# haoheliu/ssr_eval

Measured on AMD Instinct MI355X. Metric: utterance-pairs/sec (LSD+SSIM, 48kHz, n_fft=2048), higher is better.
Workload: dtype f64

## Files before the change

### ssr_eval_amd/csrc/ssr_stft_wave.h

```cpp
#pragma once
#include "ssr_stft.h"


constexpr int SSR_W_N = 2048, SSR_W_L = 64, SSR_W_P = 32;
constexpr int SSR_W_TWP = 7 * 32 + 12 * 64;
SSR_DEV int ssr_wpad(int i) { return i + (i >> 5); }
constexpr int SSR_W_PN = SSR_W_N + (SSR_W_N >> 5) + 1;

template <typename T> SSR_DEV cx<T> ssr_w32(int m) {
  constexpr double c[22] = {1.0, 0.98078528040323044913, 0.92387953251128675613, 0.83146961230254523708, 0.70710678118654752440,
                            0.55557023301960222474, 0.38268343236508977173, 0.19509032201612826785, 0.0,
                            -0.19509032201612826785, -0.38268343236508977173, -0.55557023301960222474, -0.70710678118654752440,
                            -0.83146961230254523708, -0.92387953251128675613, -0.98078528040323044913, -1.0,
                            -0.98078528040323044913, -0.92387953251128675613, -0.83146961230254523708, -0.70710678118654752440,
                            -0.55557023301960222474};
  constexpr double s[22] = {0.0, -0.19509032201612826785, -0.38268343236508977173, -0.55557023301960222474, -0.70710678118654752440,
                            -0.83146961230254523708, -0.92387953251128675613, -0.98078528040323044913, -1.0,
                            -0.98078528040323044913, -0.92387953251128675613, -0.83146961230254523708, -0.70710678118654752440,
                            -0.55557023301960222474, -0.38268343236508977173, -0.19509032201612826785, 0.0,
                            0.19509032201612826785, 0.38268343236508977173, 0.55557023301960222474, 0.70710678118654752440,
                            0.83146961230254523708};
  return {(T)c[m], (T)s[m]};
}

template <typename T, int NZ = 32> SSR_DEV void ssr_dft32(cx<T>* v) {
  const T h = (T)0.70710678118654752440;
  static_assert(NZ == 32 || (NZ > 8 && NZ <= 16), "full, or two non-zero row groups");
  SSR_UNROLL for (int n2 = 0; n2 < 8; ++n2) {
    cx<T> t[4] = {v[n2], v[8 + n2], v[16 + n2], v[24 + n2]};
    if (NZ == 32) {
      ssr_bfly4(t);
    } else if (8 + n2 < NZ) {
      const cx<T> r = cmul_negi(t[1]);
      t[2] = csub(t[0], t[1]); t[3] = csub(t[0], r);
      t[1] = cadd(t[0], r);    t[0] = cadd(t[0], v[8 + n2]);
    } else {
      t[1] = t[0]; t[2] = t[0]; t[3] = t[0];
    }
    SSR_UNROLL for (int k1 = 0; k1 < 4; ++k1) {
      const int m = n2 * k1;
      cx<T> x = t[k1];
      if (m == 0) {
      } else if (m == 8) {
        x = cmul_negi(x);
      } else if (m == 16) {
        x = {-x.x, -x.y};
      } else if (m == 4) {
        x = {h * (x.x + x.y), h * (x.y - x.x)};
      } else if (m == 12) {
        x = {h * (x.y - x.x), -h * (x.x + x.y)};
      } else if (m == 20) {
        x = {-h * (x.x + x.y), h * (x.x - x.y)};
      } else {
        x = cmul(x, ssr_w32<T>(m));
      }
      v[8 * k1 + n2] = x;
    }
  }
  SSR_UNROLL for (int k1 = 0; k1 < 4; ++k1) ssr_bfly8(v + 8 * k1);
}
SSR_DEV constexpr int ssr_dft32_freq(int rho) { return (rho >> 3) + 4 * (rho & 7); }

struct SsrTrue { static constexpr bool value = true; };
struct SsrFalse { static constexpr bool value = false; };

template <typename T, bool SUMS> struct SsrWaveRegs {
  cx<T> v[SSR_W_P];
  T tx[SSR_W_P];
  float pa[SSR_W_P], pb[SSR_W_P];
  T wl[SSR_W_P / 2];
  cx<T> tw1[3];
  cx<T> tw2[12];
  double lsd_total;
};

template <typename T, bool SPLIT> struct SsrWaveLds {
  static constexpr size_t bytes() { return sizeof(double) * 4 + sizeof(int) * 8 + sizeof(T) * (SPLIT ? 1 : 2) * SSR_W_PN; }
  double* sc1; int* nz; T* re; T* im;
  SSR_MEMBER explicit SsrWaveLds(char* base) {
    sc1 = reinterpret_cast<double*>(base);
    nz = reinterpret_cast<int*>(sc1 + 4);
    re = reinterpret_cast<T*>(nz + 8);
    im = SPLIT ? re : re + SSR_W_PN;
  }
  SSR_MEMBER bool nonzero(int which, int par) const {
    int f = nz[which * 2 + par];
#ifndef SSR_HOST_EMU
    f = __builtin_amdgcn_readfirstlane(f);
#endif
    return f != 0;
  }
};

template <typename T> struct SsrWaveBuf { T* re; T* im; };

template <typename T, bool SPLIT> constexpr size_t ssr_stft_wave_sums_offset() { return (SsrWaveLds<T, SPLIT>::bytes() + 7) & ~(size_t)7; }
template <typename T, bool SPLIT, bool SUMS> constexpr size_t ssr_stft_wave_lds_bytes() {
  return SUMS ? ssr_stft_wave_sums_offset<T, SPLIT>() + 6 * 64 * sizeof(double) : SsrWaveLds<T, SPLIT>::bytes();
}

struct SsrWaveBase { int st0, ld8, st1; };
SSR_DEV SsrWaveBase ssr_wave_bases(int tid) {
  return {33 * tid, tid + (tid >> 5), 264 * (tid >> 5) + (tid & 31)};
}
SSR_DEV constexpr int ssr_w_off_st0(int i) { return ssr_dft32_freq(i); }
SSR_DEV constexpr int ssr_w_off_ld8(int i) { return 66 * (i >> 3) + 264 * (i & 7); }
SSR_DEV constexpr int ssr_w_off_st1(int i) { return 528 * (i >> 3) + 33 * (i & 7); }

#define SSR_W_EXCHANGE_G(blk, regs, L, WB, WO, RBASES, RIDX, EXTRA)                                       \
  if constexpr (!SPLIT) {                                                                                 \
    SSR_WPHASE(blk, regs, { const int w_ = ssr_wave_bases(tid & 63).WB;                                        \
      SSR_UNROLL for (int i = 0; i < SSR_W_P; ++i) { (L).re[w_ + WO(i)] = R.v[i].x; (L).im[w_ + WO(i)] = R.v[i].y; } }); \
    SSR_WPHASE(blk, regs, { SSR_SCHED_BARRIER(); EXTRA; const auto r_ = RBASES(tid & 63);                    \
      SSR_UNROLL for (int i = 0; i < SSR_W_P; ++i) R.v[i] = {(L).re[RIDX(r_, i)], (L).im[RIDX(r_, i)]}; });   \
  } else {                                                                                                \
    SSR_WPHASE(blk, regs, { const int w_ = ssr_wave_bases(tid & 63).WB;                                        \
      SSR_UNROLL for (int i = 0; i < SSR_W_P; ++i) (L).re[w_ + WO(i)] = R.v[i].x; });                     \
    SSR_WPHASE(blk, regs, { SSR_SCHED_BARRIER(); EXTRA; const auto r_ = RBASES(tid & 63);                    \
      SSR_UNROLL for (int i = 0; i < SSR_W_P; ++i) R.tx[i] = (L).re[RIDX(r_, i)]; });                     \
    SSR_WPHASE(blk, regs, { const int w_ = ssr_wave_bases(tid & 63).WB;                                        \
      SSR_UNROLL for (int i = 0; i < SSR_W_P; ++i) (L).re[w_ + WO(i)] = R.v[i].y; });                     \
    SSR_WPHASE(blk, regs, { const auto r_ = RBASES(tid & 63);                                                \
      SSR_UNROLL for (int i = 0; i < SSR_W_P; ++i) R.v[i] = {R.tx[i], (L).re[RIDX(r_, i)]}; });           \
  }
#define SSR_W_RIDX_LD8(b_, i) ((b_).ld8 + ssr_w_off_ld8(i))
#define SSR_W_EXCHANGE(blk, regs, L, WB, WO, RB, RO, EXTRA) SSR_W_EXCHANGE_G(blk, regs, L, WB, WO, ssr_wave_bases, SSR_W_RIDX_##RB##_##RO, EXTRA)
#define SSR_W_RIDX_ld8_ssr_w_off_ld8(b_, i) SSR_W_RIDX_LD8(b_, i)

struct SsrWavePBase { int ld8, p2, p3; };
SSR_DEV int ssr_wave_pj3(int tid) { return tid == 0 ? 128 : 256 - tid; }
SSR_DEV SsrWavePBase ssr_wave_pbases(int tid) {
  return {tid + (tid >> 5), ssr_wpad(192 - tid), ssr_wpad(ssr_wave_pj3(tid))};
}
SSR_DEV int ssr_w_rd_paired(const SsrWavePBase& B, int i) {
  const int b = i >> 3, q = i & 7;
  return (b == 0 ? B.ld8 : b == 1 ? B.ld8 + 66 : b == 2 ? B.p2 : B.p3) + 264 * q;
}
#define SSR_W_RIDX_PAIRED(b_, i) ssr_w_rd_paired(b_, i)
#define SSR_W_LOAD_TW2_PAIRED { const int t_ = tid & 63; const unsigned l_ = SSR_UIDX(t_);                       \
    const unsigned o2_ = SSR_UIDX(t_ == 0 ? 192 : 64 - t_); const unsigned o3_ = SSR_UIDX(t_ == 0 ? -192 : 64 - t_); \
    SSR_UNROLL for (int i = 0; i < 6; ++i) R.tw2[i] = VT.at(l_ + (SSR_W_N + 224 + 64 * i));                       \
    SSR_UNROLL for (int i = 6; i < 9; ++i) R.tw2[i] = VT.at(o2_ + (SSR_W_N + 224 + 64 * i));                      \
    SSR_UNROLL for (int i = 9; i < 12; ++i) R.tw2[i] = VT.at(o3_ + (SSR_W_N + 224 + 64 * i)); }

#define SSR_W_LOAD_TW1 { const unsigned l_ = SSR_UIDX(tid & 31); \
                         SSR_UNROLL for (int m = 0; m < 3; ++m) R.tw1[m] = VT.at(l_ + (SSR_W_N + 32 * ((1 << m) - 1))); }
#define SSR_W_LOAD_TW2 { const unsigned l_ = SSR_UIDX(tid & 63); \
                         SSR_UNROLL for (int i = 0; i < 12; ++i) R.tw2[i] = VT.at(l_ + (SSR_W_N + 224 + 64 * i)); }
#define SSR_W_FFT_TAIL(blk, BLK0, regs, L, EXTRA2)                                                                        \
  SSR_W_FFT_TAIL_X(blk, BLK0, regs, L, SSR_W_EXCHANGE(blk, regs, L, st1, ssr_w_off_st1, ld8, ssr_w_off_ld8, SSR_W_LOAD_TW2 EXTRA2))
#define SSR_W_FFT_TAIL_PAIRED(blk, BLK0, regs, L)                                                                         \
  SSR_W_FFT_TAIL_X(blk, BLK0, regs, L, SSR_W_EXCHANGE_G(blk, regs, L, st1, ssr_w_off_st1, ssr_wave_pbases, SSR_W_RIDX_PAIRED, SSR_W_LOAD_TW2_PAIRED))
#define SSR_W_FFT_TAIL_X(blk, BLK0, regs, L, EXCH2)                                                                   \
  blk = BLK0; ssr_launder(blk);                                                                                       \
  SSR_W_EXCHANGE(blk, regs, L, st0, ssr_w_off_st0, ld8, ssr_w_off_ld8, SSR_W_LOAD_TW1);                               \
  \
  SSR_WPHASE(blk, regs, {                                                                                             \
    const cx<T> s1_ = ssr_tw_w8(R.tw1[0]);                                                                            \
    SSR_UNROLL for (int b = 0; b < 4; ++b) ssr_bfly8_tw(R.v + 8 * b, R.tw1[0], R.tw1[1], R.tw1[2], s1_);              \
  });                                                                                                                 \
  blk = BLK0; ssr_launder(blk);                                                                                       \
  EXCH2;                                                                                                              \
                     \
  SSR_WPHASE(blk, regs, {                                                                                             \
    SSR_UNROLL for (int b = 0; b < 4; ++b)                                                                            \
      ssr_bfly8_tw(R.v + 8 * b, R.tw2[3 * b], R.tw2[3 * b + 1], R.tw2[3 * b + 2], ssr_tw_w8(R.tw2[3 * b]));           \
  });

template <typename T, int WHICH = 3, typename REGS>
SSR_DEV void ssr_wave_prefetch(const SsrStftParams<T>& p, REGS& R, int tid, const SsrView<float>& va, const SsrView<float>& vb,
                               int u, int n, int n_frames) {
  const int t_c = (u < n_frames) ? u : n_frames - 1;
  const int base = t_c * p.hop - SSR_W_N / 2;
  if (base >= 0 && base + SSR_W_N <= n) {
    SSR_UNROLL for (int r = 0; r < SSR_W_P; ++r) {
      if (WHICH & 1) R.pa[r] = va.at(SSR_UIDX(tid + 64 * r), base);
      if (WHICH & 2) R.pb[r] = vb.at(SSR_UIDX(tid + 64 * r), base);
    }
  } else {
    SSR_UNROLL for (int r = 0; r < SSR_W_P; ++r) {
      const unsigned m = SSR_UIDX(ssr_reflect(base + tid + 64 * r, n));
      if (WHICH & 1) R.pa[r] = va.at(m);
      if (WHICH & 2) R.pb[r] = vb.at(m);
    }
  }
}

template <typename REGS> SSR_DEV void ssr_wave_flags(REGS& R, int tid, int* nz, int par) {
  SSR_UNROLL for (int r = 0; r < SSR_W_P; ++r) { ssr_touch(R.pa[r]); ssr_touch(R.pb[r]); }
  unsigned ora = 0u, orb = 0u;
  SSR_UNROLL for (int r = 1; r < SSR_W_P; ++r) { ora |= ssr_mag_bits(R.pa[r]); orb |= ssr_mag_bits(R.pb[r]); }
  ora |= (tid == 0) ? 0u : ssr_mag_bits(R.pa[0]);
  orb |= (tid == 0) ? 0u : ssr_mag_bits(R.pb[0]);
  SSR_WAVE_ANY_STORE(tid, ora != 0u, nz + par);
  SSR_WAVE_ANY_STORE(tid, orb != 0u, nz + 2 + par);
}

template <typename T, bool SUMS, bool SPLIT, int MAG = -1, typename BLK>
SSR_BODY void ssr_stft_wave_body(const SsrStftParams<T>& p, BLK& blk, int chunk, int item, char* lds_base) {
  constexpr int N = SSR_W_N, F = N / 2 + 1;
  using Regs = SsrWaveRegs<T, SUMS>;
  SsrWaveLds<T, SPLIT> L(lds_base);
  const int n = p.len[item], hop = p.hop;
  const int n_frames = ssr_num_frames_dev(n, N, hop);
  const int S = p.interleave > 1 ? p.interleave : 1;
  const int span0 = (chunk / S) * S * p.units_per_chunk;
  const int u0 = span0 + chunk % S;
  const int u1 = (span0 + S * p.units_per_chunk < n_frames) ? span0 + S * p.units_per_chunk : n_frames;
  const float* sa = p.a + p.a_off[item];
  const float* sb = p.b + p.b_off[item];
  const int64_t row0 = p.frame_off[item];
  double* part = p.part ? p.part + ((int64_t)item * p.n_chunks + chunk) * SSR_NPART : nullptr;
  const int mask = SUMS ? p.metric_mask : (p.metric_mask & SSR_M_LSD);
  const bool want_lsd = mask & SSR_M_LSD;
  const SsrView<float> va(sa, n), vb(sb, n);
  const SsrView<T> vw(p.window, N);
  const SsrView<cx<T>> vt(p.tw, N + SSR_W_TWP);

  double* lsum = reinterpret_cast<double*>(lds_base + ssr_stft_wave_sums_offset<T, SPLIT>());
  SSR_REGS(Regs, regs, blk);
  SSR_WPHASE(blk, regs, {
    R.lsd_total = 0.0;
    if constexpr (SUMS) for (int q = 0; q < 6; ++q) lsum[64 * q + tid] = 0.0;
    if (tid == 0) L.sc1[0] = 0.0;
    if (u0 < u1) {
      ssr_wave_prefetch<T>(p, R, tid, va, vb, u0, n, n_frames);
      SSR_UNROLL for (int r = 0; r < SSR_W_P / 2; ++r) R.wl[r] = vw.at(SSR_UIDX(tid + 64 * r));
    }
    SSR_VMEM_DRAIN();
  });

  BLK blk0 = blk;
  for (int u = u0, it = 0; u < u1; u += S, ++it) {
    blk = blk0; ssr_launder(blk);
    SSR_WPHASE(blk, regs, {
      ssr_wave_flags(R, tid, L.nz, it & 1);
      SSR_UNROLL for (int r = 0; r < SSR_W_P; ++r) {
        const T w = (r < SSR_W_P / 2) ? R.wl[r] : (T)0.5 - R.wl[r - SSR_W_P / 2];
        R.v[r] = {(T)R.pa[r] * w, (T)R.pb[r] * w};
      }
      ssr_dft32(R.v);
      if (want_lsd && it > 0 && tid == 0) R.lsd_total += sqrt(L.sc1[0] / (double)F);
    });
#define VT vt
    SSR_W_FFT_TAIL_PAIRED(blk, blk0, regs, L);
#undef VT

    blk = blk0; ssr_launder(blk);
    const int64_t OP = p.out_pitch ? p.out_pitch : F;
    float* ra0 = p.out_a ? p.out_a + (row0 + u) * OP : nullptr;
    float* rb0 = p.out_b ? p.out_b + (row0 + u) * OP : nullptr;
    SSR_WPHASE(blk, regs, {
      SSR_SCHED_BARRIER();
      double acc[7] = {0.0, 0.0, 0.0, 0.0, 0.0, 0.0, 0.0};
      const int par = it & 1;
      const bool a_nz = L.nonzero(0, par), b_nz = L.nonzero(1, par);
      const bool both = a_nz && b_nz;
      const bool store = MAG < 0 ? p.out_kind == SSR_OUT_MAG : MAG != 0;
      const SsrRwView<float> wa(ra0, store ? F : 0), wb(rb0, (store && rb0 != nullptr) ? F : 0);
      const int lane4 = 4 * tid, lane4_2 = 4 * (192 - tid), lane4_3 = 4 * ssr_wave_pj3(tid);
      auto bin_off = [&](int b, int q) -> int {
        return (b == 0 ? lane4 : b == 1 ? lane4 + 256 : b == 2 ? lane4_2 : lane4_3) + 1024 * q;
      };
      cx<T> rot4 = {(T)0, (T)0};
      if (tid == 0) {
        rot4 = R.v[28];
        const cx<T> t29 = R.v[29], t30 = R.v[30], t31 = R.v[31];
        R.v[31] = R.v[0]; R.v[30] = R.v[7]; R.v[29] = R.v[6]; R.v[28] = R.v[5];
        R.v[7] = t31; R.v[6] = t30; R.v[5] = t29;
      }
      constexpr int G = 2;
      constexpr int PF1 = SUMS ? 1 : 0;
      auto bins = [&](auto fast_tag) {
        constexpr bool FAST = decltype(fast_tag)::value;
        SSR_UNROLL for (int b = 0; b < 4; ++b) SSR_UNROLL for (int q0 = 0; q0 < 4; q0 += G) {
          cx<T> zn[G];
          SSR_UNROLL for (int q = 0; q < G; ++q) zn[q] = R.v[8 * (3 - b) + 7 - (q0 + q)];
          SSR_UNROLL for (int q = 0; q < G; q += 2) {
            const cx<T> zk0 = R.v[8 * b + q0 + q], zk1 = R.v[8 * b + q0 + q + 1];
            f2 e, t;
            if constexpr (FAST) {
              ssr_pair_bins2_fast<T, SUMS>(acc, zk0, zn[q], zk1, zn[q + 1], e, t);
            } else {
              float e0, t0, e1, t1;
              ssr_pair_bin<T, 0, true>(mask, acc, zk0, zn[q], a_nz, b_nz, e0, t0);
              ssr_pair_bin<T, 0, true>(mask, acc, zk1, zn[q + 1], a_nz, b_nz, e1, t1);
              e = f2_make(e0, e1); t = f2_make(t0, t1);
            }
            if (store) {
              wa.st_raw(bin_off(b, q0 + q), e.x);
              wa.st_raw(bin_off(b, q0 + q + 1), e.y);
              wb.st_raw(bin_off(b, q0 + q), t.x);
              wb.st_raw(bin_off(b, q0 + q + 1), t.y);
            }
          }
          if (b == 0 && q0 + G == 4) {
            if (tid == 0) {
              const cx<T> zq = R.v[4];
              float e, t;
              ssr_pair_bin<T, 0, true>(mask, acc, zq, zq, a_nz, b_nz, e, t);
              if (store) { wa.st_raw(4 * (N / 2), e); wb.st_raw(4 * (N / 2), t); }
              R.v[4] = rot4;
            }
          }
          if (b == PF1 && q0 + G == 4) {
            SSR_SCHED_BARRIER();
            ssr_wave_prefetch<T, 1>(p, R, tid, va, vb, u + S, n, n_frames);
            SSR_SCHED_BARRIER();
          }
          if (b == PF1 + 1 && q0 + G == 4) {
            SSR_SCHED_BARRIER();
            ssr_wave_prefetch<T, 2>(p, R, tid, va, vb, u + S, n, n_frames);
            SSR_SCHED_BARRIER();
          }
          if (b == PF1 + 2 && q0 + G == 4) {
            SSR_SCHED_BARRIER();
            SSR_UNROLL for (int r = 0; r < SSR_W_P / 2; ++r) R.wl[r] = vw.at(SSR_UIDX(tid + 64 * r));
            SSR_SCHED_BARRIER();
          }
        }
      };
      constexpr int FULL = SUMS ? (SSR_M_LSD | SSR_M_LOG_SISPEC | SSR_M_SISPEC) : SSR_M_LSD;
      if (both && (mask & 7) == FULL) bins(SsrTrue{});
      else bins(SsrFalse{});
      if (want_lsd) SSR_WAVE_SUM_STORE(tid, 64, acc[0], L.sc1);
      if constexpr (SUMS)
        for (int q = 0; q < 6; ++q) SSR_LDS_ACCUM(lsum + 64 * q + tid, acc[1 + q]);
    });
  }

  if (part == nullptr) return;
  if constexpr (SUMS) {
    for (int q = 0; q < 6; ++q) {
      SSR_WPHASE(blk, regs, SSR_WAVE_SUM_STORE(tid, 64, lsum[64 * q + tid], L.sc1 + 1));
      SSR_WPHASE(blk, regs, if (tid == 0) part[1 + q] = L.sc1[1]);
    }
  } else {
    SSR_WPHASE(blk, regs, if (tid == 0) for (int q = 0; q < 6; ++q) part[1 + q] = 0.0);
  }
  SSR_WPHASE(blk, regs, if (tid == 0) {
    double lsd = R.lsd_total;
    if (want_lsd && u1 > u0) lsd += sqrt(L.sc1[0] / (double)F);
    part[0] = lsd;
    part[7] = 0.0;
  });
}
```

### ssr_eval_amd/csrc/ssr_tables.h

```cpp
#pragma once
#include <cmath>
#include <cstdint>
#include <vector>

#include "ssr_block.h"

static const long double SSR_PI_L = 3.14159265358979323846264338327950288L;

inline bool ssr_is_pow2(int n) { return n > 0 && (n & (n - 1)) == 0; }
inline int ssr_ilog2(int n) { int l = 0; while ((1 << l) < n) ++l; return l; }

struct SsrEngine { bool ok; bool bluestein; int logn; int radix; int q; int m; };
inline SsrEngine ssr_pick_engine(int n_fft) {
  SsrEngine e{false, false, 0, 1, 0, 0};
  if (n_fft < 2) return e;
  e.q = n_fft;
  if (ssr_is_pow2(n_fft) && n_fft >= 256 && n_fft <= 4096) { e.ok = true; e.logn = ssr_ilog2(n_fft); return e; }
  int m = 256;
  while (m < 2 * n_fft - 1) m <<= 1;
  if (n_fft % 3 == 0 && m >= 8192) {
    const int q = n_fft / 3;
    int mq = 256;
    while (mq < 2 * q - 1) mq <<= 1;
    if (mq <= 2048) { e.ok = true; e.bluestein = true; e.logn = ssr_ilog2(mq); e.radix = 3; e.q = q; return e; }
  }
  if (m > 8192) return e;
  e.ok = true; e.bluestein = true; e.logn = ssr_ilog2(m);
  return e;
}

inline SsrEngine ssr_pick_wave_engine(int n_fft) {
  const SsrEngine e = ssr_pick_engine(n_fft);
  SsrEngine none{false, false, 0, 1, 0, 0};
  if (!e.ok || !e.bluestein) return none;
  SsrEngine w = none;
  if (e.radix == 3) w = (e.logn == 11 && e.q <= 768) ? e : none;
  else if (e.logn == 11) w = e;
  else if (e.logn == 12 && n_fft % 2 == 0 && n_fft / 2 <= 1024) w = SsrEngine{true, true, 11, 2, n_fft / 2, 0};
  if (w.ok && w.q <= 768) w.m = 1536;
  return w;
}

constexpr int SSR_WAVE_N = 2048, SSR_WAVE_TWP = 7 * 32 + 12 * 64;
constexpr int SSR_WAVE24_N = 1536, SSR_WAVE24_TWP = 2 * 9 * 64;

template <typename T> struct SsrTables {
  SsrEngine eng;
  int n_fft;
  std::vector<T> window;
  std::vector<T> window_h;
  std::vector<cx<T>> tw, wchirp, bfilt, chirp;
};

inline void ssr_host_fft_ld(std::vector<long double>& re, std::vector<long double>& im) {
  const int n = (int)re.size();
  for (int i = 1, j = 0; i < n; ++i) {
    int bit = n >> 1;
    for (; j & bit; bit >>= 1) j ^= bit;
    j ^= bit;
    if (i < j) { std::swap(re[i], re[j]); std::swap(im[i], im[j]); }
  }
  for (int len = 2; len <= n; len <<= 1) {
    for (int i = 0; i < n; i += len) {
      for (int k = 0; k < len / 2; ++k) {
        const long double ang = -2.0L * SSR_PI_L * k / len;
        const long double wr = cosl(ang), wi = sinl(ang);
        const int a = i + k, b = i + k + len / 2;
        const long double xr = re[b] * wr - im[b] * wi, xi = re[b] * wi + im[b] * wr;
        re[b] = re[a] - xr; im[b] = im[a] - xi;
        re[a] += xr; im[a] += xi;
      }
    }
  }
}

inline void ssr_host_dft_ld(std::vector<long double>& re, std::vector<long double>& im) {
  const int n = (int)re.size();
  std::vector<long double> c(n), s(n), orr(n), oi(n);
  for (int i = 0; i < n; ++i) { const long double a = -2.0L * SSR_PI_L * i / n; c[i] = cosl(a); s[i] = sinl(a); }
  for (int k = 0; k < n; ++k) {
    long double ar = 0.0L, ai = 0.0L;
    for (int m = 0; m < n; ++m) {
      const int j = (int)(((int64_t)k * m) % n);
      ar += re[m] * c[j] - im[m] * s[j];
      ai += re[m] * s[j] + im[m] * c[j];
    }
    orr[k] = ar; oi[k] = ai;
  }
  re = orr; im = oi;
}

template <typename T> bool ssr_build_tables_for(int n_fft, SsrEngine eng, SsrTables<T>& t);
template <typename T> bool ssr_build_tables(int n_fft, SsrTables<T>& t) { return ssr_build_tables_for<T>(n_fft, ssr_pick_engine(n_fft), t); }

template <typename T> bool ssr_build_tables_for(int n_fft, SsrEngine eng, SsrTables<T>& t) {
  t.eng = eng;
  t.n_fft = n_fft;
  if (!t.eng.ok) return false;
  const int N = t.eng.m ? t.eng.m : (1 << t.eng.logn);
  t.window.resize(n_fft);
  std::vector<long double> w(n_fft);
  for (int m = 0; m < n_fft; ++m) {
    w[m] = 0.5L - 0.5L * cosl(2.0L * SSR_PI_L * m / n_fft);
    t.window[m] = (T)w[m];
  }
  t.window_h.resize(n_fft);
  for (int m = 0; m < n_fft; ++m) t.window_h[m] = (T)0.5 * t.window[m];
  t.tw.resize(N);
  for (int i = 0; i < N; ++i) {
    const long double ang = -2.0L * SSR_PI_L * i / N;
    t.tw[i] = {(T)cosl(ang), (T)sinl(ang)};
  }
  if (N == SSR_WAVE24_N) {
    t.tw.resize(N + SSR_WAVE24_TWP);
    for (int b = 0; b < 3; ++b)
      for (int k = 0; k < 3; ++k)
        for (int l = 0; l < 64; ++l) {
          const int j = l + 64 * b, q = j % 24;
          t.tw[N + 64 * (3 * b + k) + l] = t.tw[(8 * q << k) % N];
          t.tw[N + 576 + 64 * (3 * b + k) + l] = t.tw[(j << k) % N];
        }
  }
  if (N == SSR_WAVE_N) {
    t.tw.resize(N + SSR_WAVE_TWP);
    for (int q = 1; q < 8; ++q)
      for (int l = 0; l < 32; ++l) t.tw[N + 32 * (q - 1) + l] = t.tw[8 * l * q];
    for (int b = 0; b < 4; ++b)
      for (int k = 0; k < 3; ++k)
        for (int l = 0; l < 64; ++l) t.tw[N + 224 + 64 * (3 * b + k) + l] = t.tw[(l + 64 * b) << k];
  }
  if (t.eng.bluestein) {
    const int q = t.eng.q, R = t.eng.radix;
    std::vector<long double> cr(q), ci(q);
    for (int k = 0; k < q; ++k) {
      const int64_t kk = ((int64_t)k * k) % (2 * (int64_t)q);
      const long double ang = -SSR_PI_L * (long double)kk / q;
      cr[k] = cosl(ang); ci[k] = sinl(ang);
    }
    t.chirp.resize((size_t)R * q); t.wchirp.resize((size_t)R * q);
    for (int r = 0; r < R; ++r)
      for (int k = 0; k < q; ++k) {
        const int64_t rk = ((int64_t)r * k) % n_fft;
        const long double a2 = -2.0L * SSR_PI_L * (long double)rk / n_fft;
        const long double tr = cosl(a2), ti = sinl(a2);
        t.chirp[(size_t)r * q + k] = {(T)(0.5L * (cr[k] * tr - ci[k] * ti)), (T)(0.5L * (cr[k] * ti + ci[k] * tr))};
        const long double wv = w[(size_t)R * k + r];
        t.wchirp[(size_t)r * q + k] = {(T)(wv * cr[k]), (T)(wv * ci[k])};
      }
    std::vector<long double> br(N, 0.0L), bi(N, 0.0L);
    for (int m = 0; m < q; ++m) {
      br[m] = cr[m]; bi[m] = -ci[m];
      if (m) { br[N - m] = cr[m]; bi[N - m] = -ci[m]; }
    }
    if (ssr_is_pow2(N)) ssr_host_fft_ld(br, bi); else ssr_host_dft_ld(br, bi);
    t.bfilt.resize(N);
    for (int i = 0; i < N; ++i) t.bfilt[i] = {(T)(br[i] / N), (T)(bi[i] / N)};
  }
  return true;
}
```

### ssr_eval_amd/csrc/tu_stft.inc

```
#include "ssr_host.h"
#include "ssr_stft_r3.h"
#include "ssr_stft_wave.h"
#include "ssr_stft_rn_wave.h"
#include "ssr_stft_r3_rot.h"

typedef SSR_TU_T TT;
static_assert(SSR_W_N == SSR_WAVE_N && SSR_W_TWP == SSR_WAVE_TWP, "ssr_tables.h appends what ssr_stft_wave.h reads");
static_assert(SSR_W24_N == SSR_WAVE24_N && SSR_W24_TWP == SSR_WAVE24_TWP, "ssr_tables.h appends what ssr_fft24.h reads");

constexpr int ssr_stft_min_waves(int logn, bool blu, bool sums) { return (logn == 11 && !blu && !sums) ? 4 : 1; }

#if SSR_TU_PART <= 2
template <typename T, int LOGN, bool BLU, int MODE, bool SUMS, int E64>
__global__ __launch_bounds__((1 << LOGN) / ssr_stft_ppt(LOGN, BLU), E64 ? 1 : ssr_stft_min_waves(LOGN, BLU, SUMS))
void k_stft(SsrStftParams<T> p) {
  extern __shared__ __attribute__((aligned(16))) char smem[];
  SsrBlk blk{(int)threadIdx.x};
  const int item = blockIdx.x / p.n_chunks, chunk = blockIdx.x % p.n_chunks;
  ssr_stft_body<T, LOGN, BLU, MODE, SUMS, ssr_stft_ppt(LOGN, BLU), E64>(p, blk, chunk, item, smem);
}

template <typename T, int LOGN, bool BLU, int MODE, bool SUMS, int E64 = 0>
static int launch_stft_mode(SsrStftParams<T>& p, int grid, hipStream_t s) {
  constexpr int PPT = ssr_stft_ppt(LOGN, BLU);
  const size_t lds = SsrStftLds<T, LOGN, PPT>::bytes();
  static thread_local SsrLdsSlot slot;
  if (int rc = ssr_allow_lds((const void*)k_stft<T, LOGN, BLU, MODE, SUMS, E64>, lds, &slot)) return rc;
  hipLaunchKernelGGL((k_stft<T, LOGN, BLU, MODE, SUMS, E64>), dim3(grid), dim3((1 << LOGN) / PPT), lds, s, p);
  HIP_TRY(hipGetLastError());
  return SSR_OK;
}

template <typename T, int LOGN, bool BLU> static int launch_stft_inst(SsrStftParams<T>& p, int grid, hipStream_t s) {
  const bool sums = p.metric_mask & (SSR_M_SISPEC | SSR_M_LOG_SISPEC);
  (void)sums;
#if SSR_TU_PART == 2
  return launch_stft_mode<T, LOGN, BLU, SSR_MODE_SINGLE, false>(p, grid, s);
#elif SSR_TU_PART == 1
  if (p.a64 && p.b64)
    return sums ? launch_stft_mode<T, LOGN, BLU, SSR_MODE_PAIR, true, SSR_IN_BOTH64>(p, grid, s)
                : launch_stft_mode<T, LOGN, BLU, SSR_MODE_PAIR, false, SSR_IN_BOTH64>(p, grid, s);
  return sums ? launch_stft_mode<T, LOGN, BLU, SSR_MODE_PAIR, true, SSR_IN_EST64>(p, grid, s)
              : launch_stft_mode<T, LOGN, BLU, SSR_MODE_PAIR, false, SSR_IN_EST64>(p, grid, s);
#else
  return sums ? launch_stft_mode<T, LOGN, BLU, SSR_MODE_PAIR, true>(p, grid, s)
              : launch_stft_mode<T, LOGN, BLU, SSR_MODE_PAIR, false>(p, grid, s);
#endif
}

#if SSR_TU_PART == 0
template <typename T, bool SUMS, bool SPLIT, bool MAG>
__global__ __launch_bounds__(64, SPLIT ? 2 : 1) void k_stft_wave(SsrStftParams<T> p, int n_groups) {
  extern __shared__ __attribute__((aligned(16))) char smem[];
  SsrBlk blk{(int)threadIdx.x};
  int logical = (int)blockIdx.x;
  if (p.interleave > 1) {
    const int S = p.interleave, xcd = (int)blockIdx.x & 7, slot = (int)blockIdx.x >> 3;
    const int G = (slot / S) * 8 + xcd;
    if (G >= n_groups) return;
    logical = G * S + slot % S;
  }
  const int item = logical / p.n_chunks, chunk = logical % p.n_chunks;
  ssr_stft_wave_body<T, SUMS, SPLIT, MAG ? 1 : 0>(p, blk, chunk, item, smem);
}
template <typename T, bool SUMS> static int launch_stft_wave(SsrStftParams<T>& p, int grid, hipStream_t s) {
  const size_t lds = ssr_stft_wave_lds_bytes<T, true, SUMS>();
  int n_groups = grid;
  if (p.interleave > 1) {
    if (p.n_chunks % p.interleave) return ssr_fail(SSR_ERR_INVALID_ARG, "interleaved chunks: n_chunks must be a multiple of the group size");
    n_groups = grid / p.interleave;
    grid = ssr_ceil_div(n_groups, 8) * 8 * p.interleave;
  }
  if (p.out_kind == SSR_OUT_MAG) hipLaunchKernelGGL((k_stft_wave<T, SUMS, true, true>), dim3(grid), dim3(64), lds, s, p, n_groups);
  else hipLaunchKernelGGL((k_stft_wave<T, SUMS, true, false>), dim3(grid), dim3(64), lds, s, p, n_groups);
  HIP_TRY(hipGetLastError());
  return SSR_OK;
}
#endif

static int launch_stft_part(const ssr_plan* pl, SsrStftParams<TT>& p, int grid, hipStream_t s) {
#if SSR_TU_PART == 0
  if (ssr_stft_uses_wave_engine(pl, false)) {
    const bool sums = p.metric_mask & (SSR_M_SISPEC | SSR_M_LOG_SISPEC);
    return sums ? launch_stft_wave<TT, true>(p, grid, s) : launch_stft_wave<TT, false>(p, grid, s);
  }
#endif
#define CASE(L)                                                                   \
  case L:                                                                         \
    return pl->eng.bluestein ? launch_stft_inst<TT, L, true>(p, grid, s) : launch_stft_inst<TT, L, false>(p, grid, s);
  switch (pl->eng.logn) { CASE(8) CASE(9) CASE(10) CASE(11) CASE(12)
    case 13: return launch_stft_inst<TT, 13, true>(p, grid, s);
  }
#undef CASE
  return ssr_fail(SSR_ERR_UNSUPPORTED, "no kernel for this FFT length");
}

#if SSR_TU_PART == 0
template <> int ssr_launch_stft_pair<TT>(const ssr_plan* pl, SsrStftParams<TT>& p, int grid, hipStream_t s) { return launch_stft_part(pl, p, grid, s); }
#elif SSR_TU_PART == 1
template <> int ssr_launch_stft_pair64<TT>(const ssr_plan* pl, SsrStftParams<TT>& p, int grid, hipStream_t s) { return launch_stft_part(pl, p, grid, s); }
#else
template <> int ssr_launch_stft_single<TT>(const ssr_plan* pl, SsrStftParams<TT>& p, int grid, hipStream_t s) { return launch_stft_part(pl, p, grid, s); }
#endif

#else
template <typename T, int LOGN, int MODE, bool SUMS, int E64>
__global__ __launch_bounds__((1 << LOGN) / 8) void k_stft_r3(SsrStftParams<T> p) {
  extern __shared__ __attribute__((aligned(16))) char smem[];
  SsrBlk blk{(int)threadIdx.x};
  const int item = blockIdx.x / p.n_chunks, chunk = blockIdx.x % p.n_chunks;
  ssr_stft_r3_body<T, LOGN, MODE, SUMS, E64>(p, blk, chunk, item, smem);
}

template <typename T, int LOGN, int MODE, bool SUMS, int E64 = 0>
static int launch_stft_r3_mode(SsrStftParams<T>& p, int grid, hipStream_t s) {
  const size_t lds = SsrStftR3Lds<T, LOGN>::bytes(p.n_fft / 3);
  static thread_local SsrLdsSlot slot;
  if (int rc = ssr_allow_lds((const void*)k_stft_r3<T, LOGN, MODE, SUMS, E64>, lds, &slot)) return rc;
  hipLaunchKernelGGL((k_stft_r3<T, LOGN, MODE, SUMS, E64>), dim3(grid), dim3((1 << LOGN) / 8), lds, s, p);
  HIP_TRY(hipGetLastError());
  return SSR_OK;
}

template <typename T, int LOGN> static int launch_stft_r3_inst(SsrStftParams<T>& p, int grid, hipStream_t s) {
  const bool sums = p.metric_mask & (SSR_M_SISPEC | SSR_M_LOG_SISPEC);
  (void)sums;
#if SSR_TU_PART == 3
  if (p.mode != SSR_MODE_PAIR) return launch_stft_r3_mode<T, LOGN, SSR_MODE_SINGLE, false>(p, grid, s);
  return sums ? launch_stft_r3_mode<T, LOGN, SSR_MODE_PAIR, true>(p, grid, s)
              : launch_stft_r3_mode<T, LOGN, SSR_MODE_PAIR, false>(p, grid, s);
#else
  if (p.a64 && p.b64)
    return sums ? launch_stft_r3_mode<T, LOGN, SSR_MODE_PAIR, true, SSR_IN_BOTH64>(p, grid, s)
                : launch_stft_r3_mode<T, LOGN, SSR_MODE_PAIR, false, SSR_IN_BOTH64>(p, grid, s);
  return sums ? launch_stft_r3_mode<T, LOGN, SSR_MODE_PAIR, true, SSR_IN_EST64>(p, grid, s)
              : launch_stft_r3_mode<T, LOGN, SSR_MODE_PAIR, false, SSR_IN_EST64>(p, grid, s);
#endif
}

#if SSR_TU_PART == 3
template <typename T, bool SUMS, int NW, int NQ, int P>
__global__ __launch_bounds__(64 * NW, (NQ == 4 && sizeof(T) == 8) ? 1 : 2) void k_stft_rn_wave(SsrStftParams<T> p) {
  extern __shared__ __attribute__((aligned(16))) char smem[];
  SsrBlk blk{(int)threadIdx.x};
  const int item = blockIdx.x / p.n_chunks, chunk = blockIdx.x % p.n_chunks;
  ssr_stft_rn_wave_body<T, SUMS, NW, NQ, P>(p, blk, chunk, item, smem);
}
template <typename T, bool SUMS, int NW, int NQ, int P> static int launch_stft_rn_wave(SsrStftParams<T>& p, int grid, hipStream_t s) {
  const size_t lds = ssr_stft_rn_wave_lds_bytes<T, NW, SUMS, P>();
  static thread_local SsrLdsSlot slot;
  if (int rc = ssr_allow_lds((const void*)k_stft_rn_wave<T, SUMS, NW, NQ, P>, lds, &slot)) return rc;
  hipLaunchKernelGGL((k_stft_rn_wave<T, SUMS, NW, NQ, P>), dim3(grid), dim3(64 * NW), lds, s, p);
  HIP_TRY(hipGetLastError());
  return SSR_OK;
}
template <typename T, int NW, int NQ, int P> static int launch_stft_rn_wave_sums(SsrStftParams<T>& p, int grid, hipStream_t s) {
  return (p.metric_mask & (SSR_M_SISPEC | SSR_M_LOG_SISPEC)) ? launch_stft_rn_wave<T, true, NW, NQ, P>(p, grid, s)
                                                             : launch_stft_rn_wave<T, false, NW, NQ, P>(p, grid, s);
}
template <typename T, bool SUMS, int NQ, int P, int IN64 = 0>
__global__ __launch_bounds__(64 * SSR_R3ROT_WAVES, 2) void k_stft_r3_rot(SsrStftParams<T> p) {
  extern __shared__ __attribute__((aligned(16))) char smem[];
  SsrBlk blk{(int)threadIdx.x};
  const int item = blockIdx.x / p.n_chunks, chunk = blockIdx.x % p.n_chunks;
  ssr_stft_r3_rot_body<T, SUMS, NQ, P, IN64>(p, blk, chunk, item, smem);
}
template <typename T, bool SUMS, int NQ, int P, int IN64 = 0> static int launch_stft_r3_rot(SsrStftParams<T>& p, int grid, hipStream_t s) {
  const size_t lds = SsrR3RotLds<T, P>::bytes(p.n_fft / 3);
  static thread_local SsrLdsSlot slot;
  if (int rc = ssr_allow_lds((const void*)k_stft_r3_rot<T, SUMS, NQ, P, IN64>, lds, &slot)) return rc;
  hipLaunchKernelGGL((k_stft_r3_rot<T, SUMS, NQ, P, IN64>), dim3(grid), dim3(64 * SSR_R3ROT_WAVES), lds, s, p);
  HIP_TRY(hipGetLastError());
  return SSR_OK;
}
template <> int ssr_launch_stft_rn_wave<TT>(const ssr_plan* pl, SsrStftParams<TT>& p, int grid, hipStream_t s) {
  const bool wide = pl->weng.q > 768;
  if (pl->weng.m == SSR_W24_N) {
    switch (ssr_stft_rn_wave_radix(pl)) {
      case 1: return launch_stft_rn_wave_sums<TT, 1, 3, 24>(p, grid, s);
      case 2: return launch_stft_rn_wave_sums<TT, 2, 3, 24>(p, grid, s);
      case 3: {
        if constexpr (sizeof(TT) == 8) {
          if (p.a64 != nullptr && p.b64 != nullptr)
            return launch_stft_r3_rot<TT, false, 3, 24, SSR_IN_EST64X2>(p, grid, s);
        }
        if (p.a64 != nullptr)
          return (p.metric_mask & (SSR_M_SISPEC | SSR_M_LOG_SISPEC)) ? launch_stft_r3_rot<TT, true, 3, 24, SSR_IN_EST64>(p, grid, s)
                                                                     : launch_stft_r3_rot<TT, false, 3, 24, SSR_IN_EST64>(p, grid, s);
        return (p.metric_mask & (SSR_M_SISPEC | SSR_M_LOG_SISPEC)) ? launch_stft_r3_rot<TT, true, 3, 24>(p, grid, s)
                                                                   : launch_stft_r3_rot<TT, false, 3, 24>(p, grid, s);
      }
    }
    return ssr_fail(SSR_ERR_UNSUPPORTED, "no wave kernel for this n_fft");
  }
  switch (ssr_stft_rn_wave_radix(pl)) {
    case 1: return wide ? launch_stft_rn_wave_sums<TT, 1, 4, 32>(p, grid, s) : launch_stft_rn_wave_sums<TT, 1, 3, 32>(p, grid, s);
    case 2: return wide ? launch_stft_rn_wave_sums<TT, 2, 4, 32>(p, grid, s) : launch_stft_rn_wave_sums<TT, 2, 3, 32>(p, grid, s);
    case 3: return launch_stft_rn_wave_sums<TT, 3, 3, 32>(p, grid, s);
  }
  return ssr_fail(SSR_ERR_UNSUPPORTED, "no wave kernel for this n_fft");
}
#endif

static int launch_stft_r3_part(const ssr_plan* pl, SsrStftParams<TT>& p, int grid, hipStream_t s) {
  switch (pl->eng.logn) {
    case 8: return launch_stft_r3_inst<TT, 8>(p, grid, s);
    case 9: return launch_stft_r3_inst<TT, 9>(p, grid, s);
    case 10: return launch_stft_r3_inst<TT, 10>(p, grid, s);
    case 11: return launch_stft_r3_inst<TT, 11>(p, grid, s);
  }
  return ssr_fail(SSR_ERR_UNSUPPORTED, "no radix-3 kernel for this FFT length");
}
#if SSR_TU_PART == 3
template <> int ssr_launch_stft_r3<TT>(const ssr_plan* pl, SsrStftParams<TT>& p, int grid, hipStream_t s) { return launch_stft_r3_part(pl, p, grid, s); }
#else
template <> int ssr_launch_stft_r3_64<TT>(const ssr_plan* pl, SsrStftParams<TT>& p, int grid, hipStream_t s) { return launch_stft_r3_part(pl, p, grid, s); }
#endif
#endif
```

Measured before the change: 363,600.

## Derive Hann window per lane from one twiddle and fold it into first DFT layer

Result: faster. 371,900, median of 6 (+2.3%).

```diff
diff --git a/ssr_eval_amd/csrc/ssr_stft_wave.h b/ssr_eval_amd/csrc/ssr_stft_wave.h
--- a/ssr_eval_amd/csrc/ssr_stft_wave.h
+++ b/ssr_eval_amd/csrc/ssr_stft_wave.h
@@ -3,7 +3,8 @@
 
 
 constexpr int SSR_W_N = 2048, SSR_W_L = 64, SSR_W_P = 32;
-constexpr int SSR_W_TWP = 7 * 32 + 12 * 64;
+constexpr int SSR_W_WCS_OFF = 7 * 32 + 12 * 64;
+constexpr int SSR_W_TWP = SSR_W_WCS_OFF + 64;
 SSR_DEV int ssr_wpad(int i) { return i + (i >> 5); }
 constexpr int SSR_W_PN = SSR_W_N + (SSR_W_N >> 5) + 1;
 
@@ -59,6 +60,58 @@
   }
   SSR_UNROLL for (int k1 = 0; k1 < 4; ++k1) ssr_bfly8(v + 8 * k1);
 }
+
+template <int M, typename T> SSR_DEV void ssr_bfly2_w32(cx<T>& a, cx<T>& b) {
+  static_assert(M > 0 && M < 16, "the exponents of ssr_bfly8_w32<1..3> are 1..15 (ssr_w32 holds 0..21)");
+  if constexpr (M == 8) { const cx<T> r = cmul_negi(b); const cx<T> p = cadd(a, r); b = csub(a, r); a = p; }
+  else ssr_bfly2_tw(a, b, ssr_w32<T>(M));
+}
+template <int K1, typename T> SSR_DEV void ssr_bfly8_w32(cx<T>* v) {
+  cx<T> a0 = v[0], a1 = v[1], a2 = v[2], a3 = v[3], b0 = v[4], b1 = v[5], b2 = v[6], b3 = v[7];
+  ssr_bfly2_w32<4 * K1>(a0, b0);
+  ssr_bfly2_w32<4 * K1>(a1, b1);
+  ssr_bfly2_w32<4 * K1>(a2, b2);
+  ssr_bfly2_w32<4 * K1>(a3, b3);
+  ssr_bfly2_w32<2 * K1>(a0, a2);
+  ssr_bfly2_w32<2 * K1>(a1, a3);
+  ssr_bfly2_w32<2 * K1 + 8>(b0, b2);
+  ssr_bfly2_w32<2 * K1 + 8>(b1, b3);
+  ssr_bfly2_w32<K1>(a0, a1);
+  ssr_bfly2_w32<K1 + 8>(a2, a3);
+  ssr_bfly2_w32<K1 + 4>(b0, b1);
+  ssr_bfly2_w32<K1 + 12>(b2, b3);
+  v[0] = a0; v[1] = b0; v[2] = a2; v[3] = b2; v[4] = a1; v[5] = b1; v[6] = a3; v[7] = b3;
+}
+template <typename T> SSR_DEV void ssr_window_from_lane(T* wl, cx<T> cs) {
+  SSR_UNROLL for (int r = 0; r < SSR_W_P / 2; ++r) {
+    const cx<T> e = ssr_w32<T>(r);
+    if (r == 0) wl[r] = (T)0.25 - cs.x;
+    else if (r == 8) wl[r] = (T)0.25 + cs.y;
+    else wl[r] = ssr_fma(-cs.y, e.y, ssr_fma(-cs.x, e.x, (T)0.25));
+  }
+}
+template <typename T> SSR_DEV void ssr_dft32_win_layer1(cx<T>* v, const float* pa, const float* pb, const T* wl) {
+  SSR_UNROLL for (int n2 = 0; n2 < 8; ++n2) {
+    const T w0 = wl[n2], w1 = wl[8 + n2], w2 = (T)0.5 - w0, w3 = (T)0.5 - w1;
+    const cx<T> x2 = {(T)pa[16 + n2], (T)pb[16 + n2]}, x3 = {(T)pa[24 + n2], (T)pb[24 + n2]};
+    const cx<T> t0 = {(T)pa[n2] * w0, (T)pb[n2] * w0}, t1 = {(T)pa[8 + n2] * w1, (T)pb[8 + n2] * w1};
+    const cx<T> b0 = {ssr_fma(x2.x, w2, t0.x), ssr_fma(x2.y, w2, t0.y)};
+    const cx<T> b1 = {ssr_fma(-x2.x, w2, t0.x), ssr_fma(-x2.y, w2, t0.y)};
+    const cx<T> b2 = {ssr_fma(x3.x, w3, t1.x), ssr_fma(x3.y, w3, t1.y)};
+    const cx<T> b3 = cmul_negi(cx<T>{ssr_fma(-x3.x, w3, t1.x), ssr_fma(-x3.y, w3, t1.y)});
+    v[n2] = cadd(b0, b2); v[8 + n2] = cadd(b1, b3); v[16 + n2] = csub(b0, b2); v[24 + n2] = csub(b1, b3);
+  }
+}
+template <typename T> SSR_DEV void ssr_dft32_win_rest(cx<T>* v) {
+  ssr_bfly8(v);
+  ssr_bfly8_w32<1>(v + 8);
+  ssr_bfly8_w32<2>(v + 16);
+  ssr_bfly8_w32<3>(v + 24);
+}
+template <typename T> SSR_DEV void ssr_dft32_win(cx<T>* v, const float* pa, const float* pb, const T* wl) {
+  ssr_dft32_win_layer1(v, pa, pb, wl);
+  ssr_dft32_win_rest(v);
+}
 SSR_DEV constexpr int ssr_dft32_freq(int rho) { return (rho >> 3) + 4 * (rho & 7); }
 
 struct SsrTrue { static constexpr bool value = true; };
@@ -68,7 +121,7 @@
   cx<T> v[SSR_W_P];
   T tx[SSR_W_P];
   float pa[SSR_W_P], pb[SSR_W_P];
-  T wl[SSR_W_P / 2];
+  cx<T> wcs;
   cx<T> tw1[3];
   cx<T> tw2[12];
   double lsd_total;
@@ -148,14 +201,18 @@
 #define SSR_W_LOAD_TW2 { const unsigned l_ = SSR_UIDX(tid & 63); \
                          SSR_UNROLL for (int i = 0; i < 12; ++i) R.tw2[i] = VT.at(l_ + (SSR_W_N + 224 + 64 * i)); }
 #define SSR_W_FFT_TAIL(blk, BLK0, regs, L, EXTRA2)                                                                        \
-  SSR_W_FFT_TAIL_X(blk, BLK0, regs, L, SSR_W_EXCHANGE(blk, regs, L, st1, ssr_w_off_st1, ld8, ssr_w_off_ld8, SSR_W_LOAD_TW2 EXTRA2))
+  SSR_W_FFT_TAIL_X(blk, BLK0, regs, L, SSR_W_LOAD_TW1, , SSR_W_EXCHANGE(blk, regs, L, st1, ssr_w_off_st1, ld8, ssr_w_off_ld8, SSR_W_LOAD_TW2 EXTRA2))
 #define SSR_W_FFT_TAIL_PAIRED(blk, BLK0, regs, L)                                                                         \
-  SSR_W_FFT_TAIL_X(blk, BLK0, regs, L, SSR_W_EXCHANGE_G(blk, regs, L, st1, ssr_w_off_st1, ssr_wave_pbases, SSR_W_RIDX_PAIRED, SSR_W_LOAD_TW2_PAIRED))
-#define SSR_W_FFT_TAIL_X(blk, BLK0, regs, L, EXCH2)                                                                   \
+  SSR_W_FFT_TAIL_X(blk, BLK0, regs, L, SSR_W_LOAD_TW1, , SSR_W_EXCHANGE_G(blk, regs, L, st1, ssr_w_off_st1, ssr_wave_pbases, SSR_W_RIDX_PAIRED, SSR_W_LOAD_TW2_PAIRED))
+#define SSR_W_FFT_TAIL_PAIRED_EARLY(blk, BLK0, regs, L)                                                                   \
+  SSR_W_FFT_TAIL_X(blk, BLK0, regs, L, , SSR_SCHED_BARRIER(); SSR_W_LOAD_TW2_PAIRED; SSR_SCHED_BARRIER(),                \
+                    SSR_W_EXCHANGE_G(blk, regs, L, st1, ssr_w_off_st1, ssr_wave_pbases, SSR_W_RIDX_PAIRED, ))
+#define SSR_W_FFT_TAIL_X(blk, BLK0, regs, L, LOAD1, EARLY2, EXCH2)                                                    \
   blk = BLK0; ssr_launder(blk);                                                                                       \
-  SSR_W_EXCHANGE(blk, regs, L, st0, ssr_w_off_st0, ld8, ssr_w_off_ld8, SSR_W_LOAD_TW1);                               \
+  SSR_W_EXCHANGE(blk, regs, L, st0, ssr_w_off_st0, ld8, ssr_w_off_ld8, LOAD1);                                        \
   \
   SSR_WPHASE(blk, regs, {                                                                                             \
+    EARLY2;                                                                                                           \
     const cx<T> s1_ = ssr_tw_w8(R.tw1[0]);                                                                            \
     SSR_UNROLL for (int b = 0; b < 4; ++b) ssr_bfly8_tw(R.v + 8 * b, R.tw1[0], R.tw1[1], R.tw1[2], s1_);              \
   });                                                                                                                 \
@@ -214,7 +271,6 @@
   const int mask = SUMS ? p.metric_mask : (p.metric_mask & SSR_M_LSD);
   const bool want_lsd = mask & SSR_M_LSD;
   const SsrView<float> va(sa, n), vb(sb, n);
-  const SsrView<T> vw(p.window, N);
   const SsrView<cx<T>> vt(p.tw, N + SSR_W_TWP);
 
   double* lsum = reinterpret_cast<double*>(lds_base + ssr_stft_wave_sums_offset<T, SPLIT>());
@@ -225,7 +281,7 @@
     if (tid == 0) L.sc1[0] = 0.0;
     if (u0 < u1) {
       ssr_wave_prefetch<T>(p, R, tid, va, vb, u0, n, n_frames);
-      SSR_UNROLL for (int r = 0; r < SSR_W_P / 2; ++r) R.wl[r] = vw.at(SSR_UIDX(tid + 64 * r));
+      R.wcs = vt.at(SSR_UIDX(tid) + (SSR_W_N + SSR_W_WCS_OFF));
     }
     SSR_VMEM_DRAIN();
   });
@@ -233,17 +289,20 @@
   BLK blk0 = blk;
   for (int u = u0, it = 0; u < u1; u += S, ++it) {
     blk = blk0; ssr_launder(blk);
+#define VT vt
     SSR_WPHASE(blk, regs, {
       ssr_wave_flags(R, tid, L.nz, it & 1);
-      SSR_UNROLL for (int r = 0; r < SSR_W_P; ++r) {
-        const T w = (r < SSR_W_P / 2) ? R.wl[r] : (T)0.5 - R.wl[r - SSR_W_P / 2];
-        R.v[r] = {(T)R.pa[r] * w, (T)R.pb[r] * w};
-      }
-      ssr_dft32(R.v);
       if (want_lsd && it > 0 && tid == 0) R.lsd_total += sqrt(L.sc1[0] / (double)F);
+      T wl[SSR_W_P / 2];
+      ssr_touch(R.wcs.x); ssr_touch(R.wcs.y);
+      ssr_window_from_lane(wl, R.wcs);
+      ssr_dft32_win_layer1(R.v, R.pa, R.pb, wl);
+      SSR_SCHED_BARRIER();
+      SSR_W_LOAD_TW1;
+      SSR_SCHED_BARRIER();
+      ssr_dft32_win_rest(R.v);
     });
-#define VT vt
-    SSR_W_FFT_TAIL_PAIRED(blk, blk0, regs, L);
+    SSR_W_FFT_TAIL_PAIRED_EARLY(blk, blk0, regs, L);
 #undef VT
 
     blk = blk0; ssr_launder(blk);
@@ -313,11 +372,6 @@
             ssr_wave_prefetch<T, 2>(p, R, tid, va, vb, u + S, n, n_frames);
             SSR_SCHED_BARRIER();
           }
-          if (b == PF1 + 2 && q0 + G == 4) {
-            SSR_SCHED_BARRIER();
-            SSR_UNROLL for (int r = 0; r < SSR_W_P / 2; ++r) R.wl[r] = vw.at(SSR_UIDX(tid + 64 * r));
-            SSR_SCHED_BARRIER();
-          }
         }
       };
       constexpr int FULL = SUMS ? (SSR_M_LSD | SSR_M_LOG_SISPEC | SSR_M_SISPEC) : SSR_M_LSD;
diff --git a/ssr_eval_amd/csrc/ssr_tables.h b/ssr_eval_amd/csrc/ssr_tables.h
--- a/ssr_eval_amd/csrc/ssr_tables.h
+++ b/ssr_eval_amd/csrc/ssr_tables.h
@@ -41,7 +41,7 @@
   return w;
 }
 
-constexpr int SSR_WAVE_N = 2048, SSR_WAVE_TWP = 7 * 32 + 12 * 64;
+constexpr int SSR_WAVE_N = 2048, SSR_WAVE_WCS_OFF = 7 * 32 + 12 * 64, SSR_WAVE_TWP = SSR_WAVE_WCS_OFF + 64;
 constexpr int SSR_WAVE24_N = 1536, SSR_WAVE24_TWP = 2 * 9 * 64;
 
 template <typename T> struct SsrTables {
@@ -128,6 +128,10 @@
     for (int b = 0; b < 4; ++b)
       for (int k = 0; k < 3; ++k)
         for (int l = 0; l < 64; ++l) t.tw[N + 224 + 64 * (3 * b + k) + l] = t.tw[(l + 64 * b) << k];
+    for (int l = 0; l < 64; ++l) {
+      const long double ang = 2.0L * SSR_PI_L * l / N;
+      t.tw[N + SSR_WAVE_WCS_OFF + l] = {(T)(0.25L * cosl(ang)), (T)(0.25L * sinl(ang))};
+    }
   }
   if (t.eng.bluestein) {
     const int q = t.eng.q, R = t.eng.radix;
diff --git a/ssr_eval_amd/csrc/tu_stft.inc b/ssr_eval_amd/csrc/tu_stft.inc
--- a/ssr_eval_amd/csrc/tu_stft.inc
+++ b/ssr_eval_amd/csrc/tu_stft.inc
@@ -5,7 +5,7 @@
 #include "ssr_stft_r3_rot.h"
 
 typedef SSR_TU_T TT;
-static_assert(SSR_W_N == SSR_WAVE_N && SSR_W_TWP == SSR_WAVE_TWP, "ssr_tables.h appends what ssr_stft_wave.h reads");
+static_assert(SSR_W_N == SSR_WAVE_N && SSR_W_TWP == SSR_WAVE_TWP && SSR_W_WCS_OFF == SSR_WAVE_WCS_OFF, "ssr_tables.h appends what ssr_stft_wave.h reads");
 static_assert(SSR_W24_N == SSR_WAVE24_N && SSR_W24_TWP == SSR_WAVE24_TWP, "ssr_tables.h appends what ssr_fft24.h reads");
 
 constexpr int ssr_stft_min_waves(int logn, bool blu, bool sums) { return (logn == 11 && !blu && !sums) ? 4 : 1; }
```
